# shacklettbp/madrona-learn

Hardware: AMD Instinct MI355X
Metric: env-steps/sec whole-node, 65536-env PPO, at 1/2/4/8 MI355X (higher is better)
Workload: dtype bf16; 1 GPU; 65536-env PPO iteration (BASELINE metric; SURVEY B8 semantics): T=32, obs=64, MLP[256,256], heads [4,8,5,5,2,2]+critic, 2 epochs x 32 minibatches of 2048 seqs (global), envs and minibatches split over 1 GPU(s); config=headline, total_envs=65536, envs_per_gpu=65536, global_minibatch_seqs=2048, minibatches_per_epoch=32, steps_per_update=32, parallelism=dp1, critic=scalar, hip_graph=True, sim_step=whole_rollout_one_launch

## Files before the change

madrona-learn_amd/csrc/ppo_rows16.h:

```cpp

#pragma once


template <int D> __device__ inline float r16_pair_dpp(float a, float b) {
    float r;
    if constexpr (D == 8)
        asm volatile(
            "s_nop 1\n\t"
            "v_add_f32_dpp %0, %1, %1 row_ror:8 row_mask:0xf bank_mask:0x3\n\t"
            "v_add_f32_dpp %0, %2, %2 row_ror:8 row_mask:0xf bank_mask:0xc"
            : "=&v"(r)
            : "v"(a), "v"(b));
    else
        asm volatile(
            "s_nop 1\n\t"
            "v_add_f32_dpp %0, %1, %1 row_ror:12 row_mask:0xf bank_mask:0x5\n\t"
            "v_add_f32_dpp %0, %2, %2 row_ror:4 row_mask:0xf bank_mask:0xa"
            : "=&v"(r)
            : "v"(a), "v"(b));
    return r;
}

__device__ inline int r16_colf(int qd, int lane) {
    const int r = lane & 15, g = lane >> 4;
    return 16 * (4 * qd + (r >> 2)) + 4 * g + (r & 3);
}
__device__ inline void r16_put_cols(float* cpl, const float (&cb)[4], const float (&cg)[4],
                                    int lane) {
#pragma unroll
    for (int qd = 0; qd < 4; ++qd) {
        const int f = r16_colf(qd, lane);
        cpl[f] = cb[qd];
        cpl[kR16H + f] = cg[qd];
    }
}

__device__ inline float r16_rowsum8(const float (&w)[8], int lane) {
    float x[4], y[2];
#pragma unroll
    for (int i = 0; i < 4; ++i) x[i] = r16_pair_dpp<4>(w[i], w[i + 4]);
    const bool h1 = (lane & 2) != 0, h0 = (lane & 1) != 0;
#pragma unroll
    for (int i = 0; i < 2; ++i) {
        const float keep = h1 ? x[i + 2] : x[i], send = h1 ? x[i] : x[i + 2];
        y[i] = keep + xlane<2>(send);
    }
    const float keep = h0 ? y[1] : y[0], send = h0 ? y[0] : y[1];
    return keep + xlane<1>(send);
}

__device__ inline float r16_dy(float z, float mean, float rstd, float gam, float bet, float da,
                               bool live, float& xh) {
    const float zc = z - mean;
    xh = zc * rstd;
    const float y = __builtin_fmaf(zc, rstd * gam, bet);
    return ((y > relu_thr<bf16>()) & live) ? da : 0.f;
}

__device__ inline void r16_dz_block(const f32x4& u, uint32_t (&zwb)[2], float mean,
                                    float rstd, float ca, float cbc, uint32_t (&dzb)[2]) {
#pragma unroll
    for (int k = 0; k < 2; ++k) {
        zwb[k] = r16_late(zwb[k]);
        const f2v zc = up_bf16(zwb[k]) - f2v{mean, mean};
        const f2v d = f2v{rstd, rstd} * f2v{u[2 * k], u[2 * k + 1]} +
                      (f2v{ca, ca} * zc + f2v{cbc, cbc});
        dzb[k] = pk_bf16(d.x, d.y);
    }
}

__device__ inline void r16_ln_bwd(f32x4 (&acc)[kR16NB], uint32_t (&zw)[kR16NB][2],
                                  float mean, float rstd, const float* gm, int g, int lane,
                                  bool live, uint32_t (&dzw)[kR16NB][2], float (&cb)[4],
                                  float (&cg)[4]) {
    mean = r16_late(mean);
    rstd = r16_late(rstd);
    float su = 0.f, sv = 0.f;
    constexpr int ord[4] = {0, 2, 1, 3};
    R16GB gb(gm, g, 0);
#pragma unroll
    for (int qd = 0; qd < kR16NB / 4; ++qd) {
        float wb[8], wg[8];
#pragma unroll
        for (int hp = 0; hp < 2; ++hp) {
            float pb[8], pg[8];
#pragma unroll
            for (int k = 0; k < 2; ++k) {
                const int step = 4 * qd + 2 * hp + k;
                const int b = 4 * qd + ord[2 * hp + k];
                float4 G, B;
                gb.take_now(b, G, B);
                const float gv[4] = {G.x, G.y, G.z, G.w}, bv[4] = {B.x, B.y, B.z, B.w};
                zw[b][0] = r16_late(zw[b][0]);
                zw[b][1] = r16_late(zw[b][1]);
#pragma unroll
                for (int i = 0; i < 4; ++i) {
                    float xh;
                    const float z = up_bf16(zw[b][i >> 1])[i & 1];
                    const float dy = r16_dy(z, mean, rstd, gv[i], bv[i], acc[b][i], live, xh);
                    const float u = dy * gv[i];
                    su += u;
                    sv = __builtin_fmaf(u, xh, sv);
                    acc[b][i] = u;
                    pb[4 * k + i] = dy;
                    pg[4 * k + i] = dy * xh;
                }
            }
            __builtin_amdgcn_sched_barrier(0);
#pragma unroll
            for (int i = 0; i < 4; ++i) {
                wb[4 * hp + i] = r16_pair_dpp<8>(pb[i], pb[4 + i]);
                wg[4 * hp + i] = r16_pair_dpp<8>(pg[i], pg[4 + i]);
            }
        }
        cb[qd] = r16_rowsum8(wb, lane);
        cg[qd] = r16_rowsum8(wg, lane);
    }
    su = add_xor32(add_xor16(su));
    sv = add_xor32(add_xor16(sv));
    const float invH = 1.0f / (float)kR16H;
    const float ca = -(rstd * rstd) * (sv * invH), cbc = -rstd * (su * invH);
#pragma unroll
    for (int b = 0; b < kR16NB; ++b) r16_dz_block(acc[b], zw[b], mean, rstd, ca, cbc, dzw[b]);
}

#ifdef ML_STAMPS
#define R16_STAMP(i) (r16_st[i] = __builtin_amdgcn_s_memtime())
#define R16_STAMPS_OUT()                                                              \
    do {                                                                              \
        if (ws.stamps && (tid & 63) == 0)                                             \
            for (int i_ = 0; i_ < 13; ++i_)                                           \
                ws.stamps[((int64_t)ptile * NT + tt) * 16 + i_] = r16_st[i_];        \
    } while (0)
#else
#define R16_STAMP(i) \
    do {             \
    } while (0)
#define R16_STAMPS_OUT() \
    do {                 \
    } while (0)
#endif

template <int DS> struct R16In {
    bf16x8 xf[DS];
    float adv, rv, vv;
    int act[2];
    float lp[2];
};

template <bool METRICS, int NW, int NT, int HC>
__global__ __launch_bounds__(64 * NW) __attribute__((amdgpu_waves_per_eu((NW + 3) / 4, (NW + 3) / 4))) void ppo_rows16_kernel(
    PolicyK P, RolloutK ro, const int32_t* __restrict__ mb_seq, int mb, int64_t M,
    const float* __restrict__ adv_st, HpK hp, WsK ws, R16Div dv) {
    extern __shared__ __attribute__((aligned(16))) char smem[];
#ifdef ML_STAMPS
    const uint64_t r16_t_entry = __builtin_amdgcn_s_memtime();
#endif
    typedef R16Lay<HC> LY;
    constexpr int LGS = LY::LGS, NHB = HC / 16;
    char* w1img = smem + LY::OffW1;
    char* whimg = smem + LY::OffWh;
    float* gb = (float*)(smem + LY::OffGb);
    float* hb = (float*)(smem + LY::OffHb);
    const float* bins = (const float*)(smem + LY::OffBins);
    const int tid = threadIdx.x;
    const int wave = __builtin_amdgcn_readfirstlane(tid >> 6);
    bf16* lgs = (bf16*)(smem + LY::OffLg) + wave * 16 * LGS;
    const int K = P.K;
    constexpr int D = kR16D, DS = D / 32;

    const int ptile = (int)blockIdx.x * NW + wave;
    auto slot_of = [&](int64_t rw, uint32_t& tl) {
        const uint32_t f = (uint32_t)rw;
        tl = r16_udiv(f, dv.mb_mag, dv.mb_sh);
        return f - tl * (uint32_t)mb;
    };
    auto srow_of = [&](int64_t rw, uint32_t seq) -> int64_t {
        uint32_t tl;
        (void)slot_of(rw, tl);
        const uint32_t c = r16_udiv(seq, dv.n_mag, dv.n_sh), b = seq - c * (uint32_t)ro.N;
        return rw < M ? ((int64_t)c * ro.bptt + tl) * ro.ld + b : 0;
    };
    const bool has_ret = ro.ret != nullptr, has_val = ro.values != nullptr;
    auto load_in = [&](int64_t sr, int ln, R16In<DS>& in) {
        const bf16* orow = (const bf16*)ro.obs + sr * D;
#pragma unroll
        for (int s = 0; s < DS; ++s)
            in.xf[s] = *(const bf16x8*)(orow + 32 * s + 8 * (ln >> 4));
        in.adv = ro.adv[sr];
        in.rv = (has_ret ? ro.ret : ro.adv)[sr];
        in.vv = (has_val ? ro.values : ro.adv)[sr];
#pragma unroll
        for (int u = 0; u < 2; ++u) {
            const int grp = (ln + 64 * u) >> 4;
            const int ga = grp < K ? grp : K - 1;
            in.act[u] = ro.actions[sr * K + ga];
            in.lp[u] = ro.logp[sr * K + ga];
        }
    };
    static_assert(NW == kR16Waves, "R16Stage stages with kR16Waves waves");
    R16In<DS> in;
    {
        uint32_t tl;
        const int64_t rw = (int64_t)ptile * (16 * NT) + (tid & 15);
        R16Stage<HC> stg;
        int tb_off = 0;
        float tb_ec = 0.f, tb_ow = 0.f;
#ifdef ML_R16_GATHER_FIRST
        load_in(srow_of(rw, (uint32_t)mb_seq[slot_of(rw, tl)]), tid & 63, in);
#else
        const uint32_t seq0 = (uint32_t)mb_seq[slot_of(rw, tl)];
#endif
        __builtin_amdgcn_sched_barrier(0);
        if (tid <= MLEARN_MAX_GROUPS) {
            tb_off = P.off[tid];
            tb_ec = tid < MLEARN_MAX_GROUPS ? hp.ecoef[tid] : 0.f;
            tb_ow = tid < MLEARN_MAX_GROUPS ? hp.objw[tid] : 0.f;
        }
        stg.load_params(P, tid);
        stg.load_images(P, tid);
#ifndef ML_R16_GATHER_FIRST
        __builtin_amdgcn_sched_barrier(0);
        load_in(srow_of(rw, r16_late(seq0)), tid & 63, in);
        __builtin_amdgcn_sched_barrier(0);
#endif
        stg.put(P, smem, tid);
        int* tab = (int*)(smem + LY::OffTab);
        if (tid <= MLEARN_MAX_GROUPS) {
            tab[tid] = tb_off;
            ((float*)tab)[MLEARN_MAX_GROUPS + 1 + tid] = tb_ec;
            ((float*)tab)[2 * (MLEARN_MAX_GROUPS + 1) + tid] = tb_ow;
        }
    }
    const float as0 = adv_st[0], as1 = adv_st[1];
    VnVals vn{hp.norm_vals != 0, {0.f, 0.f, 0.f, 0.f}};
    if (hp.norm_vals)
        for (int i = 0; i < 4; ++i) vn.v[i] = adv_st[2 + i];
    __syncthreads();
#ifdef ML_STAMPS
    const uint64_t r16_t_pro = __builtin_amdgcn_s_memtime();
#endif
    const int* t_off = (const int*)(smem + LY::OffTab);
    const float* t_ec = (const float*)t_off + MLEARN_MAX_GROUPS + 1;
    const float* t_ow = t_ec + MLEARN_MAX_GROUPS + 1;

    LossAcc m;
    bool did = false;
    uint32_t dz0w[kR16NB][2];
    float cb0[4], cg0[4];
    float* prev_cp = nullptr;
    int64_t prev_row = -1;
    const int ntask = 16 * (K + 1);
    int64_t sr_n = 0;
    constexpr bool kAhead = !METRICS;

#pragma clang loop unroll(disable)
    for (int tt = 0; tt < NT; ++tt) {
#ifdef ML_STAMPS
        uint64_t r16_st[13];
#endif
        R16_STAMP(0);
        const int lane = r16_late(tid & 63), r = lane & 15, g = lane >> 4;
        const int64_t row0 = (int64_t)ptile * (16 * NT) + 16 * tt;
        const int64_t row = row0 + r;
        const bool live = row < M;
        if (kAhead || tt == 0) {
#pragma unroll
            for (int s = 0; s < DS; ++s)
                in.xf[s] = __builtin_bit_cast(bf16x8, r16_late(__builtin_bit_cast(u4r, in.xf[s])));
            in.adv = r16_late(in.adv);
            in.rv = r16_late(in.rv);
            in.vv = r16_late(in.vv);
#pragma unroll
            for (int u = 0; u < 2; ++u) {
                in.act[u] = r16_late(in.act[u]);
                in.lp[u] = r16_late(in.lp[u]);
            }
        } else {
            load_in(sr_n, lane, in);
        }
        bf16x8 xf[DS];
#pragma unroll
        for (int s = 0; s < DS; ++s) xf[s] = in.xf[s];
        float t_adv = in.adv, rv = in.rv, vv = in.vv;
        int ract[2] = {in.act[0], in.act[1]};
        float rlp[2] = {in.lp[0], in.lp[1]};
        uint32_t seq_n = 0;
        if (tt + 1 < NT) {
            uint32_t tl;
            seq_n = (uint32_t)mb_seq[slot_of(row + 16, tl)];
        }
        auto lda0 = [&](int ln) {
            const bf16* w0 = (const bf16*)P.wt[0];
            const int rr = ln & 15, gg = ln >> 4;
            return [=](int b, int s) {
                const int n = 16 * b + rr;
                const int64_t idx = ((int64_t)(((n >> 5) * (D >> 4) + 2 * s + (gg >> 1)) * 64 +
                                               (n & 31) + 32 * (gg & 1))) * 8;
                return *(const bf16x8*)(w0 + idx);
            };
        };
        auto bf0 = [&](int s) { return xf[s]; };
        uint32_t zw0[kR16NB][2], zw[kR16NB][2], aw[kR16NB][2];
        float mean0, rstd0, mean, rstd;
        r16_fwd_layer<DS, kR16Ring0>(lda0(r16_late(lane)), bf0, zw0, mean0, rstd0);
        sr_n = srow_of(row + 16, r16_late(seq_n));
        uint32_t t_a[2];
        float t_b[2];
        {
            t_adv = r16_late(t_adv);
            rv = r16_late(rv);
            vv = r16_late(vv);
            const float retv = has_ret ? rv : t_adv + vv;
            const float ov = has_val ? vv : 0.f;
#pragma unroll
            for (int u = 0; u < 2; ++u) {
                const int grp = (lane + 64 * u) >> 4;
                t_a[u] = grp < K ? (uint32_t)r16_late(ract[u]) : __builtin_bit_cast(uint32_t, retv);
                t_b[u] = grp < K ? r16_late(rlp[u]) : ov;
            }
        }
        R16_STAMP(1);
#ifndef ML_PROBE_NO_X0
        {
            bf16* xrow = (bf16*)ws.x0 + r16_late(row) * D;
#pragma unroll
            for (int s = 0; s < DS; ++s)
                r16_st16(xrow + 32 * s + 8 * g, __builtin_bit_cast(u4r, xf[s]));
        }
#endif
        if (tt > 0) {
            r16_store_rows((bf16*)ws.dz[0] + r16_late(prev_row) * kR16H, dz0w, g);
            r16_put_cols(prev_cp, cb0, cg0, lane);
        }
        r16_ln_apply(zw0, mean0, rstd0, gb, g, aw);
        R16_STAMP(2);
        r16_fwd_layer<kR16KS, kR16Ring>(
            [&](int b, int s) { return r16_row_frag(w1img, 16 * b + r, s, g); },
            [&](int s) { return r16_bfrag(aw, s); }, zw, mean, rstd);
        R16_STAMP(3);
        if (NW > 4 && tt == 0 && wave >= NW / 2) __builtin_amdgcn_s_setprio(1);
#ifndef ML_PROBE_NO_A0
        r16_store_rows((bf16*)ws.a[0] + r16_late(row) * kR16H, aw, g);
#endif
        r16_ln_apply(zw, mean, rstd, gb + 2 * kR16H, g, aw);
        R16_STAMP(4);
        f32x4 ha[NHB];
#pragma unroll
        for (int j = 0; j < NHB; ++j) ha[j] = f32x4{0.f, 0.f, 0.f, 0.f};
        if constexpr (HC == 32) {
            r16_mm<NHB, kR16KS, 4>(
                ha, [&](int j, int s) { return r16_row_frag(whimg, 16 * j + r, s, g); },
                [&](int s) { return r16_bfrag(aw, s); });
        } else {
            const bf16* ht = (const bf16*)P.head_t;
            const uint32_t lo = r16_late((uint32_t)((r + 32 * (g & 1)) * 8 + 4 * (g >> 1)));
            r16_mm<NHB, kR16KS, kR16RingH>(
                ha,
                [&](int j, int s) {
                    const bf16* p = ht + ((j >> 1) * 8192 + s * 1024 + (j & 1) * 128);
                    const u2r a = *(const u2r*)(p + lo);
                    const u2r b = *(const u2r*)(p + 512 + lo);
                    return __builtin_bit_cast(bf16x8, u4r{a[0], a[1], b[0], b[1]});
                },
                [&](int s) { return r16_bfrag(aw, s); });
        }
        r16_store_rows((bf16*)ws.a[1] + r16_late(row) * kR16H, aw, g);
        {
            bf16* lr = lgs + r * LGS;
#pragma unroll
            for (int cbk = 0; cbk < NHB; ++cbk) {
                const int c0 = 16 * cbk + 4 * g;
                float v[4];
#pragma unroll
                for (int i = 0; i < 4; ++i) v[i] = rnd<bf16>(rnd<bf16>(ha[cbk][i]) + rnd<bf16>(hb[c0 + i]));
                *(u2r*)(lr + c0) = u2r{pk_bf16(v[0], v[1]), pk_bf16(v[2], v[3])};
            }
        }
        wave_lds_sync();
        R16_STAMP(5);
        auto loss_task = [&](int task, int act, float olp, float adv, float ret, float oval) {
            const int rr = task & 15, grp = task >> 4;
            bf16* lr = lgs + rr * LGS;
            if (row0 + rr >= M) {
                if (grp < K)
                    for (int j = t_off[grp]; j < t_off[grp + 1]; ++j) lr[j] = (bf16)0.f;
                else if (HC == 32)
                    for (int j = P.A; j < HC; ++j) lr[j] = (bf16)0.f;
                return;
            }
            if (grp < K) {
                if (hp.norm_adv) adv = (adv - as0) * as1;
                const int o0 = t_off[grp];
                loss_group(hp, lr + o0, t_off[grp + 1] - o0, act, olp, adv, t_ec[grp], t_ow[grp],
                           m);
            } else if (HC == 32) {
                loss_value(hp, lr, P.A, HC, ret, oval, m, vn);
            }
        };
        {
#pragma clang loop unroll(disable)
            for (int task = lane, u = 0; task < ntask; task += 64, ++u) {
                did = true;
                const uint32_t a = u == 0 ? t_a[0] : t_a[1];
                const float b = u == 0 ? t_b[0] : t_b[1];
                loss_task(task, (int)a, b, t_adv, __builtin_bit_cast(float, a), b);
            }
        }
        if constexpr (HC != 32) {
            wave_lds_sync();
            const uint32_t rbits = __shfl(K >= 4 ? t_a[1] : t_a[0], (16 * K + r) & 63);
            bf16* lr = lgs + r * LGS;
            const int CB = P.CB;
            if (row0 + r < M) {
                float mean;
                const float R = __builtin_bit_cast(float, rbits);
                const float vl = r16_twohot_ce(lr + P.A, CB, R, bins,
                                               hp.vcoef * hp.inv_s * hp.loss_scale, g, &mean);
                if (g == 0) {
                    const float verr = fabsf(mean - R);
                    m.svl += vl;
                    m.qvl += vl * vl;
                    m.mnvl = fminf(m.mnvl, vl);
                    m.mxvl = fmaxf(m.mxvl, vl);
                    m.serr += verr;
                    m.qerr += verr * verr;
                    m.mnerr = fminf(m.mnerr, verr);
                    m.mxerr = fmaxf(m.mxerr, verr);
                }
            } else {
                for (int j = P.A + g; j < P.A + CB; j += 4) lr[j] = (bf16)0.f;
            }
            for (int j = P.A + CB + g; j < HC; j += 4) lr[j] = (bf16)0.f;
        }
        wave_lds_sync();
        R16_STAMP(6);
        constexpr int HKS = HC / 32;
        bf16x8 dh[HKS];
#pragma unroll
        for (int s2 = 0; s2 < HKS; ++s2) {
            dh[s2] = *(const bf16x8*)(lgs + r * LGS + 32 * s2 + 8 * g);
            r16_st16((bf16*)ws.dhead + r16_late(row) * HC + 32 * s2 + 8 * g,
                     __builtin_bit_cast(u4r, dh[s2]));
        }
        float* cprow = ws.colpart + ((int64_t)ptile * NT + tt) * ws.CP;
#pragma unroll
        for (int c0 = 0; c0 < HC; c0 += 64) {
            if (c0 + lane < HC) {
                float hbs = 0.f;
#pragma unroll
                for (int rr = 0; rr < 16; ++rr) hbs += to_f32(lgs[rr * LGS + c0 + lane]);
                cprow[2 * 2 * kR16H + c0 + lane] = hbs;
            }
        }
        R16_STAMP(7);
        uint32_t dzw[kR16NB][2];
        {
            f32x4 hacc[kR16NB];
#pragma unroll
            for (int b = 0; b < kR16NB; ++b) hacc[b] = f32x4{0.f, 0.f, 0.f, 0.f};
            if constexpr (HC == 32) {
                r16_mm<kR16NB, 1, kR16Ring>(
                    hacc,
                    [&](int b, int) { return r16_tr_frag(whimg, 8 * g, 8 * g + 4, b, lane); },
                    [&](int) { return dh[0]; });
            } else {
                const bf16* hd = (const bf16*)P.head;
                const uint32_t lo = r16_late((uint32_t)((g >> 1) * 512 + (r + 32 * (g & 1)) * 8));
                r16_mm<kR16NB, HKS, kR16RingH>(
                    hacc,
                    [&](int b, int s2) {
                        const bf16* p = hd + ((b >> 1) * (HC / 16) * 512 + s2 * 1024 + (b & 1) * 128);
                        return *(const bf16x8*)(p + lo);
                    },
                    [&](int s2) { return dh[s2]; });
            }
            float cb1[4], cg1[4];
            r16_ln_bwd(hacc, zw, mean, rstd, gb + 2 * kR16H, g, lane, live, dzw, cb1, cg1);
            r16_put_cols(cprow + 2 * kR16H, cb1, cg1, lane);
        }
        r16_store_rows_keep((bf16*)ws.dz[1] + r16_late(row) * kR16H, dzw, g);
#ifndef ML_R16_AHEAD_LATE
        if (kAhead && tt + 1 < NT) {
            __builtin_amdgcn_sched_barrier(0);
            load_in(r16_late(sr_n), lane, in);
            __builtin_amdgcn_sched_barrier(0);
        } else {
            in = R16In<DS>{};
        }
#endif
        R16_STAMP(8);
        f32x4 acc[kR16NB];
#pragma unroll
        for (int b = 0; b < kR16NB; ++b) acc[b] = f32x4{0.f, 0.f, 0.f, 0.f};
        r16_mm_bm<kR16NB, kR16KS, kR16Ring>(
            acc,
            [&](int b, int s) {
                return r16_tr_frag(w1img, 32 * s + 4 * g, 32 * s + 16 + 4 * g, b, lane);
            },
            [&](int s) { return r16_bfrag(dzw, s); });
        R16_STAMP(9);
#ifdef ML_R16_AHEAD_LATE
        if (kAhead && tt + 1 < NT) {
            __builtin_amdgcn_sched_barrier(0);
            load_in(r16_late(sr_n), lane, in);
            __builtin_amdgcn_sched_barrier(0);
        } else {
            in = R16In<DS>{};
        }
#endif
        R16_STAMP(10);
        R16_STAMP(11);
        r16_ln_bwd(acc, zw0, mean0, rstd0, gb, g, lane, live, dz0w, cb0, cg0);
        prev_row = row;
        prev_cp = cprow;
        R16_STAMP(12);
        R16_STAMPS_OUT();
    }
    const int lane = tid & 63, r = lane & 15, g = lane >> 4;
    r16_store_rows((bf16*)ws.dz[0] + prev_row * kR16H, dz0w, g);
    r16_put_cols(prev_cp, cb0, cg0, lane);

#ifdef ML_STAMPS
    {
        __builtin_amdgcn_s_waitcnt(0);
        const uint64_t t_end = __builtin_amdgcn_s_memtime();
        if (ws.stamps && (tid & 63) == 0) {
            uint64_t* st = ws.stamps + (int64_t)ptile * NT * 16;
            st[13] = r16_t_entry;
            st[14] = r16_t_pro;
            st[15] = t_end;
        }
    }
#endif
    if (METRICS) {
        const float vals[kLossSlots] = {m.sobj, m.qobj, m.mnobj, m.mxobj, m.svl, m.qvl, m.mnvl,
                                        m.mxvl, m.serr, m.qerr, m.mnerr, m.mxerr, m.sent, m.qent,
                                        m.mnent, m.mxent, m.sentw, m.sobjw, 0.f, 0.f};
        constexpr int kUsed = 18;
        double* lp = ws.loss_part + (int64_t)ptile * kLossSlots;
        if (__any(did)) {
#pragma unroll
            for (int s = 0; s < kUsed; ++s) {
                const int kind = (s < 16) ? (s & 3) : 0;
                float v = vals[s];
                v = kind == 2 ? wave_reduce<2>(v) : (kind == 3 ? wave_reduce<3>(v) : wave_reduce<0>(v));
                if (lane == 0) lp[s] = v;
            }
            if (lane >= kUsed && lane < kLossSlots) lp[lane] = 0.0;
        } else if (lane < kLossSlots) {
            const int kind = (lane < 16) ? (lane & 3) : 0;
            lp[lane] = kind == 2 ? 3.4e38 : (kind == 3 ? -3.4e38 : 0.0);
        }
    }
}

struct R16Cfg {
    int nw, nt;
};
static R16Cfg rows16_cfg(int64_t Mp) {
    const int cus = device_cus();
    const int64_t kCUs = cus > 0 ? cus : 256;
    if (Mp % 256 == 0 && Mp / 256 >= kCUs) return R16Cfg{8, 2};
    if (Mp == 128 * kCUs) return R16Cfg{8, 1};
    return R16Cfg{0, 0};
}
static bool rows16_eligible(const PolicyK& P, int64_t Mp, int HC, int L, int H, bool bf) {
    const bool head = (HC == 32 && P.CB == 1) || (HC == 96 && P.CB > 1 && P.CB <= 64);
    return bf && H == kR16H && L == 2 && head && P.D == kR16D && P.K + 1 <= 8 &&
           rows16_cfg(Mp).nw > 0;
}

template <int NW, int NT, int HC>
static void launch_rows16_cfg(const PolicyK& P, const RolloutK& R, const int32_t* mb_seq, int mb,
                              int64_t M, const float* adv_st, const HpK& hp, const WsK& ws,
                              const R16Div& dv, hipStream_t s) {
    constexpr int lds = (int)R16Lay<HC>::Lds;
    if (set_lds_attr((const void*)ppo_rows16_kernel<true, NW, NT, HC>, lds, "ppo_rows16") ||
        set_lds_attr((const void*)ppo_rows16_kernel<false, NW, NT, HC>, lds, "ppo_rows16"))
        return;
    const int grid = (int)(ws.Mp / (16 * NW * NT));
    if (hp.metrics)
        hipLaunchKernelGGL((ppo_rows16_kernel<true, NW, NT, HC>), dim3(grid), dim3(64 * NW), lds,
                           s, P, R, mb_seq, mb, M, adv_st, hp, ws, dv);
    else
        hipLaunchKernelGGL((ppo_rows16_kernel<false, NW, NT, HC>), dim3(grid), dim3(64 * NW), lds,
                           s, P, R, mb_seq, mb, M, adv_st, hp, ws, dv);
}

static void launch_rows16(const PolicyK& P, const RolloutK& R, const int32_t* mb_seq, int mb,
                          int64_t M, const float* adv_st, const HpK& hp, const WsK& ws,
                          hipStream_t s) {
    R16Div dv;
    r16_magic((uint32_t)mb, dv.mb_mag, dv.mb_sh);
    r16_magic((uint32_t)R.N, dv.n_mag, dv.n_sh);
    const R16Cfg c = rows16_cfg(ws.Mp);
    if (P.HC == 32) {
        if (c.nt == 2)
            launch_rows16_cfg<8, 2, 32>(P, R, mb_seq, mb, M, adv_st, hp, ws, dv, s);
        else
            launch_rows16_cfg<8, 1, 32>(P, R, mb_seq, mb, M, adv_st, hp, ws, dv, s);
    } else {
        if (c.nt == 2)
            launch_rows16_cfg<8, 2, 96>(P, R, mb_seq, mb, M, adv_st, hp, ws, dv, s);
        else
            launch_rows16_cfg<8, 1, 96>(P, R, mb_seq, mb, M, adv_st, hp, ws, dv, s);
    }
}
```

madrona-learn_amd/csrc/r16_common.h:

```cpp
#pragma once

#include "common.h"
#include "dists.h"
#include "rowtile.h"

namespace ml {

constexpr int kR16Waves = 8;
constexpr int kR16Tiles = 2;
constexpr int kR16H = 256;
constexpr int kR16NB = kR16H / 16;
constexpr int kR16KS = kR16H / 32;
constexpr int kR16HC = MLEARN_HEAD_COLS;
constexpr int kR16D = 64;
constexpr int kR16LGS = 40;
#ifndef ML_R16_RING
#define ML_R16_RING 6
#endif
#ifndef ML_R16_RING0
#define ML_R16_RING0 16
#endif
constexpr int kR16Ring = ML_R16_RING;
constexpr int kR16Ring0 = ML_R16_RING0;
#ifndef ML_R16_RINGH
#define ML_R16_RINGH 8
#endif
constexpr int kR16RingH = ML_R16_RINGH;
constexpr int kR16TabN = 3 * (MLEARN_MAX_GROUPS + 1);
template <int HC> struct R16Lay {
    static_assert(HC == 32 || HC == 96, "head width");
    static constexpr int LGS = HC == 32 ? kR16LGS : 104;
    static constexpr size_t OffW1 = 0;
    static constexpr size_t OffWh = OffW1 + (size_t)kR16H * 512;
    static constexpr size_t OffGb = OffWh + (HC == 32 ? (size_t)HC * 512 : 0);
    static constexpr size_t OffHb = OffGb + (size_t)2 * 2 * kR16H * 4;
    static constexpr size_t OffBins = OffHb + (size_t)HC * 4;
    static constexpr size_t OffLg = OffBins + (HC == 32 ? 0 : (size_t)64 * 4);
    static constexpr size_t OffTab = OffLg + (size_t)kR16Waves * 16 * LGS * 2;
    static constexpr size_t Lds = OffTab + (size_t)kR16TabN * 4;
    static_assert(Lds <= 160 * 1024, "row-split LDS budget");
};

typedef float f2v __attribute__((ext_vector_type(2)));
typedef short short4r __attribute__((ext_vector_type(4)));
typedef __attribute__((ext_vector_type(4))) uint32_t u4r;
typedef __attribute__((ext_vector_type(2))) uint32_t u2r;

__device__ inline uint32_t r16_off(int n, int u) {
    const int sw = ((n & 7) << 2) | (((n >> 3) & 1) << 1);
    return (uint32_t)(n * 512 + ((u ^ sw) << 3));
}

template <typename V> __device__ inline V r16_late(V v) {
    asm volatile("" : "+v"(v));
    return v;
}

__device__ inline f32x4 mma16(bf16x8 a, bf16x8 b, f32x4 c) {
    return __builtin_amdgcn_mfma_f32_16x16x32_bf16(a, b, c, 0, 0, 0);
}

__device__ inline bf16x8 r16_row_frag(const char* img, int n, int s, int g) {
    const u2r lo = *(const u2r*)(img + r16_off(n, 8 * s + g));
    const u2r hi = *(const u2r*)(img + r16_off(n, 8 * s + 4 + g));
    const u4r v = {lo[0], lo[1], hi[0], hi[1]};
    return __builtin_bit_cast(bf16x8, v);
}

__device__ inline bf16x8 r16_tr_frag(const char* img, int rlo, int rhi, int b, int lane) {
    const int q = (lane >> 2) & 3, p = lane & 3;
    typedef __attribute__((address_space(3))) short4r* lp;
    const short4r lo = __builtin_amdgcn_ds_read_tr16_b64_v4i16(
        (lp)(img + (rlo & ~15) * 512 + r16_off((rlo & 15) + q, 4 * b + p)));
    const short4r hi = __builtin_amdgcn_ds_read_tr16_b64_v4i16(
        (lp)(img + (rhi & ~15) * 512 + r16_off((rhi & 15) + q, 4 * b + p)));
    typedef short short8r __attribute__((ext_vector_type(8)));
    const short8r v = {lo[0], lo[1], lo[2], lo[3], hi[0], hi[1], hi[2], hi[3]};
    return __builtin_bit_cast(bf16x8, v);
}

__device__ inline void r16_st16(void* p, u4r v) { *(u4r*)p = v; }

__device__ inline uint32_t pk_bf16(float a, float b) {
    typedef __bf16 bf16x2 __attribute__((ext_vector_type(2)));
    const bf16x2 v = {(bf16)a, (bf16)b};
    return __builtin_bit_cast(uint32_t, v);
}
__device__ inline f2v up_bf16(uint32_t w) {
    return f2v{__builtin_bit_cast(float, w << 16), __builtin_bit_cast(float, w & 0xffff0000u)};
}
__device__ inline bf16x8 r16_bfrag(const uint32_t (&w)[kR16NB][2], int s) {
    const u4r v = {w[2 * s][0], w[2 * s][1], w[2 * s + 1][0], w[2 * s + 1][1]};
    return __builtin_bit_cast(bf16x8, v);
}

template <int NBO, int NS, int RING, typename LDA, typename BF>
__device__ inline void r16_mm(f32x4 (&acc)[NBO], LDA lda, BF bfrag) {
    constexpr int N = NS * NBO;
    constexpr int RG = RING < N ? RING : N;
    __builtin_amdgcn_sched_barrier(0);
    bf16x8 ra[RG];
#pragma unroll
    for (int i = 0; i < RG; ++i) ra[i] = lda(i % NBO, i / NBO);
    bf16x8 bfr = bfrag(0);
#pragma unroll
    for (int i = 0; i < N; ++i) {
        const bf16x8 a = ra[i % RG];
        if (i + RG < N) ra[i % RG] = lda((i + RG) % NBO, (i + RG) / NBO);
        __builtin_amdgcn_sched_barrier(0);
        acc[i % NBO] = mma16(a, bfr, acc[i % NBO]);
        __builtin_amdgcn_sched_barrier(0);
        if ((i + 1) % NBO == 0 && i + 1 < N) bfr = bfrag((i + 1) / NBO);
    }
}

template <int NBO, int NS, int RING, typename LDA, typename BF>
__device__ inline void r16_mm_bm(f32x4 (&acc)[NBO], LDA lda, BF bfrag) {
    static_assert(NBO % 2 == 0, "block pairs");
    constexpr int N = NS * NBO;
    constexpr int RG = RING < N ? RING : N;
    auto jof = [](int i) { return 2 * (i / (2 * NS)) + (i & 1); };
    auto sof = [](int i) { return (i >> 1) % NS; };
    __builtin_amdgcn_sched_barrier(0);
    bf16x8 ra[RG];
#pragma unroll
    for (int i = 0; i < RG; ++i) ra[i] = lda(jof(i), sof(i));
#pragma unroll
    for (int i = 0; i < N; ++i) {
        const bf16x8 a = ra[i % RG];
        if (i + RG < N) ra[i % RG] = lda(jof(i + RG), sof(i + RG));
        __builtin_amdgcn_sched_barrier(0);
        acc[jof(i)] = mma16(a, bfrag(sof(i)), acc[jof(i)]);
        __builtin_amdgcn_sched_barrier(0);
    }
}

template <int NS, int RING, typename LDA, typename BF>
__device__ inline void r16_fwd_layer(LDA lda, BF bfrag, uint32_t (&zw)[kR16NB][2], float& mean_o,
                                     float& rstd_o) {
    f2v s2 = {0.f, 0.f}, q2 = {0.f, 0.f};
#pragma unroll
    for (int h = 0; h < 2; ++h) {
        f32x4 acc[8];
#pragma unroll
        for (int j = 0; j < 8; ++j) acc[j] = f32x4{0.f, 0.f, 0.f, 0.f};
        r16_mm<8, NS, RING>(acc, [&](int j, int s) { return lda(8 * h + j, s); }, bfrag);
#pragma unroll
        for (int j = 0; j < 8; ++j)
#pragma unroll
            for (int k = 0; k < 2; ++k) {
                zw[8 * h + j][k] = pk_bf16(acc[j][2 * k], acc[j][2 * k + 1]);
                const f2v x = up_bf16(zw[8 * h + j][k]);
                s2 += x;
                q2 = x * x + q2;
            }
    }
    float sum = s2.x + s2.y, sq = q2.x + q2.y;
    sum = add_xor32(add_xor16(sum));
    sq = add_xor32(add_xor16(sq));
    const float invH = 1.0f / (float)kR16H;
    const float mean = sum * invH;
    const float var = fmaxf(sq * invH - mean * mean, 0.f);
    mean_o = mean;
    rstd_o = rsqrtf(var + 1e-6f);
}

__device__ inline void r16_store_rows(bf16* rowp, uint32_t (&w)[kR16NB][2], int g) {
#pragma unroll
    for (int c = 0; c < kR16NB / 2; ++c) {
#pragma unroll
        for (int k = 0; k < 2; ++k) {
            const auto v = __builtin_amdgcn_permlane16_swap(w[2 * c][k], w[2 * c + 1][k], false,
                                                            false);
            w[2 * c][k] = v[0];
            w[2 * c + 1][k] = v[1];
        }
        const int blk = 2 * c + (g & 1);
        r16_st16(rowp + 16 * blk + 8 * (g >> 1),
                 u4r{w[2 * c][0], w[2 * c][1], w[2 * c + 1][0], w[2 * c + 1][1]});
    }
}

__device__ inline void r16_store_rows_keep(bf16* rowp, const uint32_t (&w)[kR16NB][2], int g) {
#pragma unroll
    for (int c = 0; c < kR16NB / 2; ++c) {
        uint32_t t[2][2];
#pragma unroll
        for (int k = 0; k < 2; ++k) {
            const auto v = __builtin_amdgcn_permlane16_swap(w[2 * c][k], w[2 * c + 1][k], false,
                                                            false);
            t[0][k] = v[0];
            t[1][k] = v[1];
        }
        const int blk = 2 * c + (g & 1);
        r16_st16(rowp + 16 * blk + 8 * (g >> 1), u4r{t[0][0], t[0][1], t[1][0], t[1][1]});
    }
}

struct R16GB {
    const float* gm;
    int g;
    float4 G, B;
    __device__ R16GB(const float* gm_, int g_, int first) : gm(gm_), g(g_) { load(first); }
    __device__ void load(int b) {
        const int f0 = r16_late(16 * b + 4 * g);
        G = *(const float4*)(gm + f0);
        B = *(const float4*)(gm + kR16H + f0);
    }
    __device__ void take_now(int b, float4& Go, float4& Bo) {
        __builtin_amdgcn_sched_barrier(0);
        load(b);
        Go = G;
        Bo = B;
    }
    __device__ void take(int following, float4& Go, float4& Bo) {
        __builtin_amdgcn_sched_barrier(0);
        Go = G;
        Bo = B;
        if (following >= 0) load(following);
    }
};

__device__ inline void r16_ln_apply(uint32_t (&zw)[kR16NB][2], float mean, float rstd,
                                    const float* gm, int g, uint32_t (&aw)[kR16NB][2]) {
    const f2v m2 = {mean, mean}, r2 = {rstd, rstd};
    R16GB gb(gm, g, 0);
#pragma unroll
    for (int b = 0; b < kR16NB; ++b) {
        float4 G, B;
        gb.take(b + 1 < kR16NB ? b + 1 : -1, G, B);
        zw[b][0] = r16_late(zw[b][0]);
        zw[b][1] = r16_late(zw[b][1]);
        const f2v y0 = __builtin_elementwise_fma(up_bf16(zw[b][0]) - m2, r2 * f2v{G.x, G.y},
                                                 f2v{B.x, B.y});
        const f2v y1 = __builtin_elementwise_fma(up_bf16(zw[b][1]) - m2, r2 * f2v{G.z, G.w},
                                                 f2v{B.z, B.w});
        aw[b][0] = pk_bf16(fmaxf(y0.x, 0.f), fmaxf(y0.y, 0.f));
        aw[b][1] = pk_bf16(fmaxf(y1.x, 0.f), fmaxf(y1.y, 0.f));
    }
}

struct R16Div {
    uint32_t mb_mag, n_mag;
    int mb_sh, n_sh;
};
__device__ inline uint32_t r16_udiv(uint32_t n, uint32_t mag, int sh) {
    return (__umulhi(n, mag) + n) >> sh;
}


template <int HC = kR16HC> struct R16Stage {
    typedef R16Lay<HC> LY;
    static constexpr int N1 = kR16H * kR16H * 2 / 16 / (64 * kR16Waves);
    u4r v1[N1], vh[2];
    float pv[2], hbv;
    __device__ inline void load_images(const PolicyK& P, int tid) {
        const u4r* src1 = (const u4r*)P.wt[1];
        const u4r* srch = (const u4r*)P.head_t;
#pragma unroll
        for (int i = 0; i < N1; ++i) v1[i] = src1[tid + i * 64 * kR16Waves];
        if (HC == 32)
#pragma unroll
            for (int i = 0; i < 2; ++i) vh[i] = srch[tid + i * 64 * kR16Waves];
    }
    __device__ inline void load_params(const PolicyK& P, int tid) {
#pragma unroll
        for (int i = 0; i < 2; ++i) {
            const int j = tid + i * 64 * kR16Waves, l = j >> 9, c = j & 511;
            pv[i] = c < kR16H ? P.lns[l][c] : P.lnb[l][c - kR16H];
        }
        hbv = tid < HC ? P.head_b[tid] : 0.f;
    }
    __device__ inline void put(const PolicyK& P, char* smem, int tid) const {
        char* w1img = smem + LY::OffW1;
        char* whimg = smem + LY::OffWh;
        float* gb = (float*)(smem + LY::OffGb);
        float* hb = (float*)(smem + LY::OffHb);
        auto put1 = [&](char* img, int U, u4r v) {
            const int n = ((U >> 10) << 5) | (U & 31), h = (U >> 5) & 1, s16 = (U >> 6) & 15;
            *(u2r*)(img + r16_off(n, 4 * s16 + h)) = u2r{v[0], v[1]};
            *(u2r*)(img + r16_off(n, 4 * s16 + 2 + h)) = u2r{v[2], v[3]};
        };
#pragma unroll
        for (int i = 0; i < N1; ++i) put1(w1img, tid + i * 64 * kR16Waves, v1[i]);
        if (HC == 32)
#pragma unroll
            for (int i = 0; i < 2; ++i) put1(whimg, tid + i * 64 * kR16Waves, vh[i]);
#pragma unroll
        for (int i = 0; i < 2; ++i) gb[tid + i * 64 * kR16Waves] = pv[i];
        if (tid < HC) hb[tid] = hbv;
        if (HC != 32 && tid < P.CB)
            ((float*)(smem + LY::OffBins))[tid] = twohot_bin(tid, P.CB);
    }
};
template <int HC = kR16HC>
__device__ inline void r16_stage(const PolicyK& P, char* smem, int tid) {
    R16Stage<HC> st;
    st.load_images(P, tid);
    st.load_params(P, tid);
    st.put(P, smem, tid);
}

__device__ inline bf16x8 r16_head_l2(const bf16* head_t, int n, int s, int g) {
    const int64_t base =
        ((int64_t)(((n >> 5) * 16 + 2 * s) * 64 + (n & 31) + 32 * (g & 1))) * 8 + 4 * (g >> 1);
    const u2r lo = *(const u2r*)(head_t + base);
    const u2r hi = *(const u2r*)(head_t + base + 512);
    const u4r v = {lo[0], lo[1], hi[0], hi[1]};
    return __builtin_bit_cast(bf16x8, v);
}

__device__ inline float r16_twohot_ce(bf16* lr, int CB, float R, const float* bins, float scale,
                                      int g, float* mean_out) {
    float cle = 0.f, cgt = 0.f;
    for (int j = g; j < CB; j += 4) {
        cle += bins[j] <= R ? 1.f : 0.f;
        cgt += bins[j] > R ? 1.f : 0.f;
    }
    cle += __shfl_xor(cle, 16);
    cle += __shfl_xor(cle, 32);
    cgt += __shfl_xor(cgt, 16);
    cgt += __shfl_xor(cgt, 32);
    const int lo = min(max((int)cle - 1, 0), CB - 1);
    const int up = min(max(CB - (int)cgt, 0), CB - 1);
    const bool same = lo == up;
    const float dl = same ? 1.f : fabsf(bins[lo] - R);
    const float du = same ? 1.f : fabsf(bins[up] - R);
    const float tot = dl + du;
    const float wl = dl / tot, wu = du / tot;
    float mx = -3.4e38f;
    for (int j = g; j < CB; j += 4) mx = fmaxf(mx, to_f32(lr[j]));
    mx = fmaxf(mx, __shfl_xor(mx, 16));
    mx = fmaxf(mx, __shfl_xor(mx, 32));
    float se = 0.f;
    for (int j = g; j < CB; j += 4) se += __expf(to_f32(lr[j]) - mx);
    se += __shfl_xor(se, 16);
    se += __shfl_xor(se, 32);
    const int mid = (CB - 1) / 2;
    float acc = 0.f;
    for (int i = g; i < mid; i += 4) {
        const int a = mid - 1 - i, b = mid + 1 + i;
        acc += (__expf(to_f32(lr[a]) - mx) / se) * bins[a] +
               (__expf(to_f32(lr[b]) - mx) / se) * bins[b];
    }
    acc += __shfl_xor(acc, 16);
    acc += __shfl_xor(acc, 32);
    *mean_out = (__expf(to_f32(lr[mid]) - mx) / se) * bins[mid] + acc;
    const float lse = mx + __logf(se);
    const float llo = to_f32(lr[lo]), lup = to_f32(lr[up]);
    const float loss = -(wl * (llo - lse) + wu * (lup - lse));
    const float wsum = wl + wu;
    for (int j = g; j < CB; j += 4) {
        const float pj = __expf(to_f32(lr[j]) - mx) / se;
        const float w = (j == lo ? wl : 0.f) + (j == up ? wu : 0.f);
        lr[j] = (bf16)((wsum * pj - w) * scale);
    }
    return loss;
}

__device__ inline float r16_twohot_mean(const bf16* lr, int CB, const float* bins, int g) {
    float mx = -3.4e38f;
    for (int j = g; j < CB; j += 4) mx = fmaxf(mx, to_f32(lr[j]));
    mx = fmaxf(mx, __shfl_xor(mx, 16));
    mx = fmaxf(mx, __shfl_xor(mx, 32));
    float se = 0.f;
    for (int j = g; j < CB; j += 4) se += __expf(to_f32(lr[j]) - mx);
    se += __shfl_xor(se, 16);
    se += __shfl_xor(se, 32);
    const int mid = (CB - 1) / 2;
    float acc = 0.f;
    for (int i = g; i < mid; i += 4) {
        const int a = mid - 1 - i, b = mid + 1 + i;
        acc += (__expf(to_f32(lr[a]) - mx) / se) * bins[a] +
               (__expf(to_f32(lr[b]) - mx) / se) * bins[b];
    }
    acc += __shfl_xor(acc, 16);
    acc += __shfl_xor(acc, 32);
    return (__expf(to_f32(lr[mid]) - mx) / se) * bins[mid] + acc;
}

static inline void r16_magic(uint32_t d, uint32_t& mag, int& sh) {
    int l = 0;
    while ((1ull << l) < d) ++l;
    mag = (uint32_t)(((1ull << 32) * ((1ull << l) - d)) / d + 1);
    sh = l;
}

}
```

Measured before the change: 241.2 million env-steps/s.

## Stage shared weights with a subset of waves and defer barrier for others

Only the first kR16StageWaves waves load the layer-1 and head weight images, LayerNorm params and tables into LDS. The remaining waves load their inputs and run the first-layer forward (which reads weights from global) before joining the workgroup barrier, so prologue staging overlaps with compute. A raw s_barrier replaces __syncthreads, late waves lower their priority on the last tile, and the GB offset is hoisted. Staging waves now carry more registers and loads each, and the split barrier relies on the non-stagers not touching LDS before they arrive.

```diff
diff --git a/madrona-learn_amd/csrc/ppo_rows16.h b/madrona-learn_amd/csrc/ppo_rows16.h
--- a/madrona-learn_amd/csrc/ppo_rows16.h
+++ b/madrona-learn_amd/csrc/ppo_rows16.h
@@ -148,6 +148,8 @@
     float lp[2];
 };
 
+constexpr int kR16StageWaves = 4;
+
 template <bool METRICS, int NW, int NT, int HC>
 __global__ __launch_bounds__(64 * NW) __attribute__((amdgpu_waves_per_eu((NW + 3) / 4, (NW + 3) / 4))) void ppo_rows16_kernel(
     PolicyK P, RolloutK ro, const int32_t* __restrict__ mb_seq, int mb, int64_t M,
@@ -198,48 +200,68 @@
             in.lp[u] = ro.logp[sr * K + ga];
         }
     };
-    static_assert(NW == kR16Waves, "R16Stage stages with kR16Waves waves");
+    static_assert(NW == kR16Waves && kR16StageWaves < NW, "some of the kR16Waves waves stage");
+    constexpr int NSW = kR16StageWaves;
+    const bool stager = wave < NSW;
+#ifdef ML_STAMPS
+    uint64_t r16_t_arr = 0, r16_t_pro = 0, r16_t_iss = 0;
+#endif
+    auto wg_barrier = [&]() {
+#ifdef ML_STAMPS
+        asm volatile("s_waitcnt lgkmcnt(0)" ::: "memory");
+        r16_t_arr = __builtin_amdgcn_s_memtime();
+        asm volatile("s_barrier" ::: "memory");
+        r16_t_pro = __builtin_amdgcn_s_memtime();
+#else
+        asm volatile("s_waitcnt lgkmcnt(0)\n\ts_barrier" ::: "memory");
+#endif
+    };
     R16In<DS> in;
     {
         uint32_t tl;
         const int64_t rw = (int64_t)ptile * (16 * NT) + (tid & 15);
-        R16Stage<HC> stg;
+        R16Stage<HC, NSW> stg;
         int tb_off = 0;
         float tb_ec = 0.f, tb_ow = 0.f;
-#ifdef ML_R16_GATHER_FIRST
-        load_in(srow_of(rw, (uint32_t)mb_seq[slot_of(rw, tl)]), tid & 63, in);
-#else
         const uint32_t seq0 = (uint32_t)mb_seq[slot_of(rw, tl)];
-#endif
         __builtin_amdgcn_sched_barrier(0);
-        if (tid <= MLEARN_MAX_GROUPS) {
-            tb_off = P.off[tid];
-            tb_ec = tid < MLEARN_MAX_GROUPS ? hp.ecoef[tid] : 0.f;
-            tb_ow = tid < MLEARN_MAX_GROUPS ? hp.objw[tid] : 0.f;
-        }
-        stg.load_params(P, tid);
-        stg.load_images(P, tid);
-#ifndef ML_R16_GATHER_FIRST
-        __builtin_amdgcn_sched_barrier(0);
-        load_in(srow_of(rw, r16_late(seq0)), tid & 63, in);
-        __builtin_amdgcn_sched_barrier(0);
-#endif
-        stg.put(P, smem, tid);
-        int* tab = (int*)(smem + LY::OffTab);
-        if (tid <= MLEARN_MAX_GROUPS) {
-            tab[tid] = tb_off;
-            ((float*)tab)[MLEARN_MAX_GROUPS + 1 + tid] = tb_ec;
-            ((float*)tab)[2 * (MLEARN_MAX_GROUPS + 1) + tid] = tb_ow;
+        if (stager) {
+            if (tid <= MLEARN_MAX_GROUPS) {
+                tb_off = P.off[tid];
+                tb_ec = tid < MLEARN_MAX_GROUPS ? hp.ecoef[tid] : 0.f;
+                tb_ow = tid < MLEARN_MAX_GROUPS ? hp.objw[tid] : 0.f;
+            }
+            stg.load_params(P, tid);
+            stg.load_images(P, tid);
+            __builtin_amdgcn_sched_barrier(0);
+            load_in(srow_of(rw, r16_late(seq0)), tid & 63, in);
+            __builtin_amdgcn_sched_barrier(0);
+#ifdef ML_STAMPS
+#ifdef ML_STAMPS_LANDING
+            asm volatile("s_waitcnt vmcnt(9)" ::: "memory");
+#endif
+            r16_t_iss = __builtin_amdgcn_s_memtime();
+#endif
+            stg.put(P, smem, tid);
+            int* tab = (int*)(smem + LY::OffTab);
+            if (tid <= MLEARN_MAX_GROUPS) {
+                tab[tid] = tb_off;
+                ((float*)tab)[MLEARN_MAX_GROUPS + 1 + tid] = tb_ec;
+                ((float*)tab)[2 * (MLEARN_MAX_GROUPS + 1) + tid] = tb_ow;
+            }
+        } else {
+            load_in(srow_of(rw, r16_late(seq0)), tid & 63, in);
+            __builtin_amdgcn_sched_barrier(0);
+#ifdef ML_STAMPS
+            r16_t_iss = __builtin_amdgcn_s_memtime();
+#endif
         }
     }
     const float as0 = adv_st[0], as1 = adv_st[1];
     VnVals vn{hp.norm_vals != 0, {0.f, 0.f, 0.f, 0.f}};
     if (hp.norm_vals)
         for (int i = 0; i < 4; ++i) vn.v[i] = adv_st[2 + i];
-    __syncthreads();
-#ifdef ML_STAMPS
-    const uint64_t r16_t_pro = __builtin_amdgcn_s_memtime();
-#endif
+    if (stager) wg_barrier();
     const int* t_off = (const int*)(smem + LY::OffTab);
     const float* t_ec = (const float*)t_off + MLEARN_MAX_GROUPS + 1;
     const float* t_ow = t_ec + MLEARN_MAX_GROUPS + 1;
@@ -260,6 +282,7 @@
         uint64_t r16_st[13];
 #endif
         R16_STAMP(0);
+        if (NW > 4 && NT > 1 && tt == NT - 1 && wave >= NW / 2) __builtin_amdgcn_s_setprio(0);
         const int lane = r16_late(tid & 63), r = lane & 15, g = lane >> 4;
         const int64_t row0 = (int64_t)ptile * (16 * NT) + 16 * tt;
         const int64_t row = row0 + r;
@@ -304,6 +327,7 @@
         uint32_t zw0[kR16NB][2], zw[kR16NB][2], aw[kR16NB][2];
         float mean0, rstd0, mean, rstd;
         r16_fwd_layer<DS, kR16Ring0>(lda0(r16_late(lane)), bf0, zw0, mean0, rstd0);
+        if (tt == 0 && !stager) wg_barrier();
         sr_n = srow_of(row + 16, r16_late(seq_n));
         uint32_t t_a[2];
         float t_b[2];
@@ -530,6 +554,10 @@
             st[13] = r16_t_entry;
             st[14] = r16_t_pro;
             st[15] = t_end;
+            if (NT > 1) {
+                st[16 + 13] = r16_t_arr;
+                st[16 + 14] = r16_t_iss;
+            }
         }
     }
 #endif
diff --git a/madrona-learn_amd/csrc/r16_common.h b/madrona-learn_amd/csrc/r16_common.h
--- a/madrona-learn_amd/csrc/r16_common.h
+++ b/madrona-learn_amd/csrc/r16_common.h
@@ -199,11 +199,13 @@
 
 struct R16GB {
     const float* gm;
-    int g;
+    int o;
     float4 G, B;
-    __device__ R16GB(const float* gm_, int g_, int first) : gm(gm_), g(g_) { load(first); }
+    __device__ R16GB(const float* gm_, int g, int first) : gm(gm_), o(r16_late(4 * g)) {
+        load(first);
+    }
     __device__ void load(int b) {
-        const int f0 = r16_late(16 * b + 4 * g);
+        const int f0 = 16 * b + o;
         G = *(const float4*)(gm + f0);
         B = *(const float4*)(gm + kR16H + f0);
     }
@@ -249,24 +251,30 @@
 }
 
 
-template <int HC = kR16HC> struct R16Stage {
+template <int HC = kR16HC, int NSW = kR16Waves> struct R16Stage {
     typedef R16Lay<HC> LY;
-    static constexpr int N1 = kR16H * kR16H * 2 / 16 / (64 * kR16Waves);
-    u4r v1[N1], vh[2];
-    float pv[2], hbv;
+    static constexpr int NTH = 64 * NSW;
+    static constexpr int N1 = kR16H * kR16H * 2 / 16 / NTH;
+    static constexpr int NH = 32 * kR16H * 2 / 16 / NTH;
+    static constexpr int NP = 2 * 2 * kR16H / NTH;
+    static_assert(N1 * NTH == kR16H * kR16H / 8 && NH * NTH == 32 * kR16H / 8 &&
+                      NP * NTH == 4 * kR16H && HC <= NTH && 64 <= NTH,
+                  "the staging threads divide the images and cover the head bias and bins");
+    u4r v1[N1], vh[NH];
+    float pv[NP], hbv;
     __device__ inline void load_images(const PolicyK& P, int tid) {
         const u4r* src1 = (const u4r*)P.wt[1];
         const u4r* srch = (const u4r*)P.head_t;
 #pragma unroll
-        for (int i = 0; i < N1; ++i) v1[i] = src1[tid + i * 64 * kR16Waves];
+        for (int i = 0; i < N1; ++i) v1[i] = src1[tid + i * NTH];
         if (HC == 32)
 #pragma unroll
-            for (int i = 0; i < 2; ++i) vh[i] = srch[tid + i * 64 * kR16Waves];
+            for (int i = 0; i < NH; ++i) vh[i] = srch[tid + i * NTH];
     }
     __device__ inline void load_params(const PolicyK& P, int tid) {
 #pragma unroll
-        for (int i = 0; i < 2; ++i) {
-            const int j = tid + i * 64 * kR16Waves, l = j >> 9, c = j & 511;
+        for (int i = 0; i < NP; ++i) {
+            const int j = tid + i * NTH, l = j >> 9, c = j & 511;
             pv[i] = c < kR16H ? P.lns[l][c] : P.lnb[l][c - kR16H];
         }
         hbv = tid < HC ? P.head_b[tid] : 0.f;
@@ -282,12 +290,12 @@
             *(u2r*)(img + r16_off(n, 4 * s16 + 2 + h)) = u2r{v[2], v[3]};
         };
 #pragma unroll
-        for (int i = 0; i < N1; ++i) put1(w1img, tid + i * 64 * kR16Waves, v1[i]);
+        for (int i = 0; i < N1; ++i) put1(w1img, tid + i * NTH, v1[i]);
         if (HC == 32)
 #pragma unroll
-            for (int i = 0; i < 2; ++i) put1(whimg, tid + i * 64 * kR16Waves, vh[i]);
-#pragma unroll
-        for (int i = 0; i < 2; ++i) gb[tid + i * 64 * kR16Waves] = pv[i];
+            for (int i = 0; i < NH; ++i) put1(whimg, tid + i * NTH, vh[i]);
+#pragma unroll
+        for (int i = 0; i < NP; ++i) gb[tid + i * NTH] = pv[i];
         if (tid < HC) hb[tid] = hbv;
         if (HC != 32 && tid < P.CB)
             ((float*)(smem + LY::OffBins))[tid] = twohot_bin(tid, P.CB);
```

New measurement: 252.5 million env-steps/s (median of 6 runs). 4.7% higher.
